# HKU-BAL/MegaPath

Hardware: NVIDIA B200
Metric: read pairs aligned/sec (higher is better)
Workload: dtype int16/u8 (integer DP, 2-bit FM-index)

## Files before the change

megapath_b200/csrc/mp_align.cu:

```cuda
#include "mp_context.h"
#include "mp_cigar.h"
#include <cub/device/device_scan.cuh>
#include <algorithm>
#include <tuple>
#include <string.h>
#include <stdlib.h>

int mps_upload(mp_context *ctx, const uint32_t *queries, const uint32_t *readLengths, uint32_t nReads, uint32_t wpq);
int mps_download_seedpos(mp_context *ctx, mp_seed_pos **readPos, uint64_t *nReadPos, mp_seed_pos **matePos, uint64_t *nMatePos);


__device__ __forceinline__ void account_work(unsigned long long cells, unsigned long long tasks, unsigned long long *__restrict__ counters)
{
#pragma unroll
    for (int d = 16; d; d >>= 1) { cells += __shfl_xor_sync(0xffffffffu, cells, d); tasks += __shfl_xor_sync(0xffffffffu, tasks, d); }
    if ((threadIdx.x & 31) == 0 && tasks) { atomicAdd(&counters[11], cells); atomicAdd(&counters[12], tasks); }
}

__global__ void k_left_tasks(const mp_candidate *__restrict__ cands, uint32_t n, const uint32_t *__restrict__ lens,
                             uint64_t fullLen, int strandLeft, MpDpTask *__restrict__ tasks, unsigned long long *__restrict__ counters)
{
    uint32_t c = blockIdx.x * blockDim.x + threadIdx.x;
    if (c >= n) { account_work(0, 0, counters); return; }
    mp_candidate ci = cands[c];
// ... 494 lines not shown

extern "C" int mp_align_pairs(mp_context *ctx, const mp_align_params *params, mp_results *out)
{
    if (!ctx || !params || !out) { mp_set_error("mp_align_pairs: null argument"); return MP_ERR_ARG; }
    if (!ctx->hasIndex || !ctx->hasBatch) { mp_set_error("mp_align_pairs: index and batch must be loaded first"); return MP_ERR_STATE; }
    if (params->matchScore != 1 || params->extendGapScore != -1 || params->mismatchScore > -2 || params->mismatchScore <= params->openGapScore * 2 ||
        params->mismatchScore < -4 || params->openGapScore < -6 || params->openGapScore >= -1) {
        mp_set_error("mp_align_pairs: score parameters outside the supported range (CPU_DP.cpp:199-208; mismatch = -1 divides by zero at CPU_DP.cpp:310, and for mismatch == 2 * open the reference traceback prefers I over D where the plain recurrence ties: unpinned, refused)"); return MP_ERR_ARG;
    }
    if ((int64_t)ctx->maxLenBatch >= (int64_t)params->maxReadLength) {
        mp_set_error("the batch holds a read of %u bases but maxReadLength is %d (reads must be shorter)", ctx->maxLenBatch, params->maxReadLength);
        return MP_ERR_ARG;
    }
    MP_CUDA(cudaSetDevice(ctx->device));
    const double wall0 = mp_now_ms();
    MpTrace tr;
    memset(out, 0, sizeof *out);
    ctx->resValid = false; ctx->fmtReady = false;
    ctx->hPairs.clear(); ctx->hRescued.clear(); ctx->hSingles.clear(); ctx->hCigars.clear();
    ctx->evUsed = 0;
    MP_CUDA(cudaEventRecord(ctx->ev[4], ctx->stream));
    if (!ctx->seeded) { if (int rc = mp_seed_pairs(ctx, params)) return rc; }
    MP_CUDA(cudaEventRecord(ctx->ev[5], ctx->stream));
    tr.mark("seed_pairs");
    uint64_t cells = 0, tasksRun = 0;
    if (int rc = deep_dp(ctx, params, out, cells, tasksRun)) return rc;
    tr.mark("deep_dp");
    if (int rc = mps_single_and_rescue(ctx, params, out, cells, tasksRun)) return rc;
    MP_CUDA(cudaEventRecord(ctx->ev[6], ctx->stream));
    unsigned long long hc[16];
    MP_CUDA(cudaMemcpyAsync(hc, ctx->dCounters.p, sizeof hc, cudaMemcpyDeviceToHost, ctx->stream));
    MP_CUDA(cudaStreamSynchronize(ctx->stream));
    tr.mark("single+default dp");
    mp_stats &S = ctx->stats;
    memset(&S, 0, sizeof S);
    S.n_occ = hc[2]; S.n_lf = hc[5] + hc[8]; S.n_sa = hc[3]; S.n_lkt = hc[4]; S.n_probe = hc[9]; S.n_text = hc[10];
    ctx->ev_collect(S.ms_fill, S.ms_tb, S.ms_exact);
    S.dp_cells = cells; S.dp_tasks = tasksRun; S.dp_tasks_exact = hc[14]; S.dp_cells_filled = hc[15];
    cudaEventElapsedTime(&S.ms_seed, ctx->ev[0], ctx->ev[1]);
    cudaEventElapsedTime(&S.ms_sa, ctx->ev[1], ctx->ev[2]);
    cudaEventElapsedTime(&S.ms_pair, ctx->ev[2], ctx->ev[3]);
    cudaEventElapsedTime(&S.ms_dp, ctx->ev[5], ctx->ev[6]);
    cudaEventElapsedTime(&S.ms_total, ctx->ev[4], ctx->ev[6]);
    out->pairs = ctx->hPairs.data(); out->n_pairs = ctx->hPairs.size();
    out->rescued = ctx->hRescued.data(); out->n_rescued = ctx->hRescued.size();
    out->singles = ctx->hSingles.data(); out->n_singles = ctx->hSingles.size();
    out->cigars = ctx->hCigars.data(); out->cigar_bytes = ctx->hCigars.size();
    ctx->seeded = false;
    ctx->resCount[0] = out->n_pairs; ctx->resCount[1] = out->n_rescued; ctx->resCount[2] = out->n_singles; ctx->resValid = true;
    if (ctx->resultsOnDevice) {
        out->pairs = nullptr; out->rescued = nullptr; out->singles = nullptr; out->cigars = nullptr;
        out->n_pairs = out->n_rescued = out->n_singles = out->cigar_bytes = 0;
    }
    S.ms_wall = (float)(mp_now_ms() - wall0);
    tr.mark("finish");
    return 0;
}
extern "C" int mp_results_on_device(mp_context *ctx, int on)
{
    if (!ctx) { mp_set_error("mp_results_on_device: null argument"); return MP_ERR_ARG; }
    ctx->resultsOnDevice = on != 0;
    return 0;
}
extern "C" int mp_last_stats(mp_context *ctx, mp_stats *stats)
{
    if (!ctx || !stats) { mp_set_error("mp_last_stats: null argument"); return MP_ERR_ARG; }
// ... 11 lines not shown
```

megapath_b200/csrc/mp_dp.cu:

```cuda
#include "mp_context.h"
#include "mp_cigar.h"
#include <cub/device/device_scan.cuh>
#include <algorithm>
#include <type_traits>

#ifndef MP_FILL_MINBLOCKS
#define MP_FILL_MINBLOCKS 6
#endif
#define DP_BIAS   0x4000
#define DP_BIAS2  0x40004000u
#define DP_NEG2   0x20C020C0u
#define DP_C      0x5000
#define DP_C2     0x50005000u
#define DP_CM1_2  0x4FFF4FFFu

__device__ __forceinline__ int h0_value(int j, int clipLt, int open)
{
    return j <= clipLt ? 0 : open - (j - clipLt - 1);
}
__device__ __forceinline__ uint32_t pack2(int v) { return ((uint32_t)v & 0xffffu) * 0x00010001u; }
__device__ __forceinline__ uint32_t prmt(uint32_t a, uint32_t b, uint32_t sel)
{
    uint32_t d; asm("prmt.b32 %0, %1, %2, %3;" : "=r"(d) : "r"(a), "r"(b), "r"(sel)); return d;
}
// ... 303 lines not shown
#pragma unroll 1
        for (int t = 1; t <= stepsR; ) {
            if (t > rampEnd && t <= steadyEnd) {
#pragma unroll 1
                for (; t <= steadyEnd; t += 4) group(t, std::false_type());
            } else { group(t, std::true_type()); t += 4; }
        }
    }
    __syncwarp();
#pragma unroll
    for (int half = 0; half < 2; ++half) {
        const int lb = tr.lb[half], thr = tr.thr[half];
        int gbest = lb;
#pragma unroll
        for (int dlt = 16; dlt; dlt >>= 1) gbest = max(gbest, __shfl_xor_sync(0xffffffffu, gbest, dlt));
        uint32_t key = 0xffffffffu, c2 = 0u;
        if (lb == gbest && gbest >= thr && tr.elig[half])
            dp_resolve_lane<K>(tables + (size_t)(blockIdx.x * 8 + (threadIdx.x >> 5) * 2) * tableStride + half * 128, S, (int)(threadIdx.x & 31) * K + 1, tr.elig[half], tr.rfirst[half], tr.rlast[half], (gbest - DP_BIAS) >> 2, key, c2);
#ifdef MP_DEBUG_TRACK
        if (pairId == 0 && half == 0) printf("dbg lane %d lb %d gbest %d thr %d thrT %d elig %x r0 %d r1 %d T2 %x N %d L %d partial %d key %x\n", lane, lb, gbest, thr, tr.thrT[0], tr.elig[0], tr.rfirst[0], tr.rlast[0], T2, NA, LA, (int)partial, key);
        if (lb == gbest && gbest >= thr && tr.elig[half] && (key == 0xffffffffu || tr.rfirst[half] < 1 || tr.rlast[half] > (half ? NB : NA)))
            printf("track: pair %u half %d lane %d gbest %d thr %d lb %d r0 %d r1 %d N %d L %d elig %x key %x cnt %u partial %d\n", pairId, half, lane, gbest, thr, lb,
                   tr.rfirst[half], tr.rlast[half], half ? NB : NA, half ? LB : LA, tr.elig[half], key, c2, (int)partial);
#endif
#pragma unroll
        for (int dlt = 16; dlt; dlt >>= 1) { key = min(key, __shfl_xor_sync(0xffffffffu, key, dlt)); c2 += __shfl_xor_sync(0xffffffffu, c2, dlt); }
        if (lane == 0 && (half == 0 || hasB)) {
            FillOut f; f.score = (gbest - DP_BIAS) >> 2; f.row = key >> 12; f.col = key & 0xfffu; f.cnt = c2;
            if (gbest < thr || !(half ? okB : okA) || key == 0xffffffffu) { f.score = 0; f.row = 0; f.col = 0; f.cnt = 0; }
            fill[half == 0 ? tA : tB] = f;
        }
    }
}

template <int K, bool WORDPAT>
__global__ void __launch_bounds__(128)
k_dp_tb(const uint8_t *__restrict__ refSeq, const uint32_t *__restrict__ refLens, uint32_t refStride,
        const uint8_t *__restrict__ readSeq, const uint32_t *__restrict__ readLens, uint32_t readStride,
        const int32_t *__restrict__ cutoffs, uint32_t taskBase, uint32_t nTasks, MpDpParams P,
        const uint8_t *__restrict__ tables, size_t tableStride, int S, const FillOut *__restrict__ fill,
        MpDpOut *__restrict__ outs, uint8_t *__restrict__ patterns, uint32_t patStride,
        const uint32_t *__restrict__ active, const uint32_t *__restrict__ nActive)
{
    const uint32_t lt = blockIdx.x * blockDim.x + threadIdx.x;
    if (active) nTasks = *nActive;
    if (lt >= nTasks) return;
    const uint32_t task = taskBase + (active ? active[lt] : lt);
    const int L = (int)readLens[task], cutoff = cutoffs[task];
    const int mm = P.mismatch, open = P.open, ext = -1, clipLt = P.clipLt;
    MpDpOut o; memset(&o, 0, sizeof o);
    const FillOut f = fill[task];
    if (cutoff > L || cutoff <= 0 || L >= 255 + open - 1 + cutoff || L > 32 * K || f.score < cutoff) { outs[task] = o; return; }
    const uint8_t *tab = tables + (size_t)(lt & ~1u) * tableStride + (lt & 1u) * 128;
    uint8_t *pat = patterns + (size_t)task * patStride;
    uint32_t tabW = 0; size_t tabIdx = ~(size_t)0;
    auto cellAt = [&](int r, int c) -> uint32_t {
        const size_t off = cell_offset<K>(r, c, S);
        if ((off >> 2) != tabIdx) { tabIdx = off >> 2; tabW = __ldcs((const uint32_t *)tab + tabIdx); }
        return (tabW >> ((off & 3) * 8)) & 0xffu;
    };
    auto flagAt = [&](int r, int c) -> int {
        if (c == 0) return 0;
        if (r == 0) return c <= clipLt ? 0 : 1;
        return trace_flag(cellAt(r, c));
    };
    auto hmodAt = [&](int r, int c) -> int {
        if (r == 0) return h0_value(c, clipLt, open) & 63;
        if (c == 0) return 0;
        return trace_h(cellAt(r, c));
    };
    const size_t rsOff = (size_t)task * readStride, fsOff = (size_t)task * refStride;
    uint32_t rsW = 0, fsW = 0; size_t rsIdx = ~(size_t)0, fsIdx = ~(size_t)0;
    auto readBase = [&](int x) -> uint32_t {
        const size_t a = rsOff + x;
        if ((a >> 2) != rsIdx) { rsIdx = a >> 2; rsW = __ldg((const uint32_t *)readSeq + rsIdx); }
        return (rsW >> ((a & 3) * 8)) & 0xffu;
    };
    auto refBase = [&](int x) -> uint32_t {
        const size_t a = fsOff + x;
        if ((a >> 2) != fsIdx) { fsIdx = a >> 2; fsW = __ldg((const uint32_t *)refSeq + fsIdx); }
        return (fsW >> ((a & 3) * 8)) & 0xffu;
    };
    uint32_t p = 0, pacc = 0;
    auto emit = [&](uint32_t byte) {
        if (WORDPAT) {
            pacc |= byte << ((p & 3) * 8);
            if ((p & 3) == 3) { ((uint32_t *)pat)[p >> 2] = pacc; pacc = 0; }
        } else pat[p] = (uint8_t)byte;
        ++p;
    };
    int cgType = 'N', cgCnt = 0, cgLast = 'N', cgLen = 0, cgI = 0, cgD = 0, cgS = 0, cgGap = 0;
    bool cgStored = P.cigText != 0;
    uint8_t *cw = pat + patStride;
    auto cgFlush = [&]() {
        if (cgCnt > 0 && cgType != 'N') {
            const int nd = ndigits(cgCnt);
            cgLen += nd + 1;
            if (cgType == 'I') cgI += cgCnt; else if (cgType == 'D') cgD += cgCnt; else if (cgType == 'S') cgS += cgCnt;
            if (cgType == 'I' || cgType == 'D') cgGap += open + (cgCnt - 1) * ext;
            if (cgStored) {
                if (cw - (nd + 1) < pat + p + 8) cgStored = false;
                else { *--cw = (uint8_t)cgType; int v = cgCnt; for (int d = 0; d < nd; ++d) { *--cw = (uint8_t)('0' + v % 10); v /= 10; } }
            }
        }
    };
    auto cgEvent = [&](int type, int cnt) { if (type == cgType) cgCnt += cnt; else { cgFlush(); cgType = type; cgCnt = cnt; } };
    auto sym = [&](uint32_t ch) { emit(ch); cgEvent((int)ch, 1); cgLast = (int)ch; };
    auto rep = [&](uint32_t c) { emit('V'); emit(c & 0xffu); cgEvent(cgLast, (int)(c & 0xffu) - 1); };
    const int hitRow = (int)f.row, hitCol = (int)f.col;
    o.score = f.score; o.count = min(f.cnt, 255u);
    int clipR = L - hitCol;
    if (clipR > 0) { sym('S'); rep((uint32_t)clipR); }
    int i = L - clipR, j = hitRow;
    enum { NORMAL, I_EXT, D_EXT, SM_EXIT, SI_EXIT, SD_EXIT };
    int state = NORMAL;
    int accum = 0;
    uint32_t cell = cellAt(j, i);
    while (i > 0 && j > 0) {
        const int flag = trace_flag(cell), hcur = trace_h(cell);
        if (state == NORMAL) {
            uint32_t diagCell = 0; int dflag, hdiag;
            if (i - 1 == 0) { dflag = 0; hdiag = 0; }
            else if (j - 1 == 0) { dflag = (i - 1) <= clipLt ? 0 : 1; hdiag = h0_value(i - 1, clipLt, open) & 63; }
            else { diagCell = cellAt(j - 1, i - 1); dflag = trace_flag(diagCell); hdiag = trace_h(diagCell); }
            const int dd = trace_diff(hcur, hdiag);
            bool eq = refBase(j - 1) == readBase(i - 1);
            int ms = eq ? 1 : mm;
            if (dd == ms) {
                if (i != 1 && dflag == 0) { state = SM_EXIT; break; }
                sym(eq ? 'M' : 'm'); --j; --i;
                cell = diagCell;
                continue;
            } else if (flag == 1) {
                int vd = trace_diff(hcur, hmodAt(j - 1, i));
                sym('D'); --j;
                if (vd != open) { accum = (int8_t)(vd - ext); state = D_EXT; }
            } else {
                int hd = trace_diff(hcur, hmodAt(j, i - 1));
                sym('I'); --i;
                if (hd != open) { accum = (int8_t)(hd - ext); state = I_EXT; }
            }
        } else if (state == D_EXT) {
            int vd = trace_diff(hcur, hmodAt(j - 1, i));
            if (vd + accum == open && flagAt(j - 1, i) == 0) { state = SD_EXIT; break; }
            sym('D'); --j;
            if (vd + accum == open) state = NORMAL; else accum = (int8_t)(accum + vd - ext);
        } else {
            int hd = trace_diff(hcur, hmodAt(j, i - 1));
            if (hd + accum == open && flagAt(j, i - 1) == 0) { state = SI_EXIT; break; }
            sym('I'); --i;
            if (hd + accum == open) state = NORMAL; else accum = (int8_t)(accum + hd - ext);
        }
        if (i > 0 && j > 0) cell = cellAt(j, i);
    }
    bool discard = false;
    if (j == 0) {
        int sc = min(clipLt & 0xff, i);
        if (sc < i) { sym('I'); rep((uint32_t)(i - sc)); }
        sym('S'); rep((uint32_t)sc);
    } else if (state == SI_EXIT) {
        sym('I'); sym('S'); rep((uint32_t)(i - 1));
    } else if (state == SD_EXIT) {
        sym('D'); sym('S'); rep((uint32_t)(i - 1));
        discard = true;
    } else if (state == SM_EXIT) {
        sym((refBase(j - 1) == readBase(i - 1)) ? 'M' : 'm');
        sym('S'); rep((uint32_t)(i - 1));
        j -= 1;
    }
    o.patLen = p;
    emit(0);
    if (WORDPAT && (p & 3)) ((uint32_t *)pat)[p >> 2] = pacc;
    cgFlush();
    if (cw < pat + p + 8) cgStored = false;
    o.cigLen = (uint16_t)cgLen; o.nI = (uint16_t)cgI; o.nD = (uint16_t)cgD; o.nS = (uint16_t)cgS; o.gapPenalty = (int16_t)cgGap; o.cigStored = cgStored ? 1 : 0;
    if (discard) { o.score = 0; o.hitLoc = 0; } else o.hitLoc = (uint32_t)j;
    outs[task] = o;
}

template <int K>
__global__ void __launch_bounds__(128)
k_dp_exact(const uint8_t *__restrict__ refSeq, const uint32_t *__restrict__ refLens, uint32_t refStride,
           const uint8_t *__restrict__ readSeq, const uint32_t *__restrict__ readLens, uint32_t readStride,
           const int32_t *__restrict__ cutoffs, uint32_t taskBase, uint32_t nTasks, MpDpParams P,
           MpDpOut *__restrict__ outs, uint8_t *__restrict__ patterns, uint32_t patStride, uint32_t *__restrict__ needDp)
{
    const int lane = threadIdx.x & 31;
    const uint32_t lt = blockIdx.x * 4 + (threadIdx.x >> 5);
    if (lt >= nTasks) return;
    const uint32_t task = taskBase + lt;
    const int N = (int)refLens[task], L = (int)readLens[task], cutoff = cutoffs[task];
    const bool ok = !(cutoff > L || cutoff <= 0 || L >= 255 + P.open - 1 + cutoff || L > 32 * K) && L > 0 && N >= L &&
                    P.mismatch <= 0 && P.open <= 0;
    uint32_t occ = 0; int first = -1;
    if (ok) {
        const uint8_t *fs = refSeq + (size_t)task * refStride, *rs = readSeq + (size_t)task * readStride;
        const int shifts = N - L + 1;
        const int PRE = L < 8 ? L : 8;
        for (int base = 0; base < shifts; base += 32) {
            const int o = base + lane;
            bool alive = o < shifts;
#pragma unroll
            for (int k = 0; k < 8; ++k)
                if (alive && k < PRE) alive = fs[o + k] == rs[k];
            uint32_t cand = __ballot_sync(0xffffffffu, alive);
            while (cand) {
                const int oc = base + __ffs(cand) - 1;
                cand &= cand - 1;
                bool same = true;
                for (int k = PRE + lane; k < L; k += 32) same = same && fs[oc + k] == rs[k];
                if (__all_sync(0xffffffffu, same)) { if (first < 0) first = oc; ++occ; }
            }
        }
    }
    if (occ == 0) { if (lane == 0) needDp[lt] = 1; return; }
    uint8_t *pat = patterns + (size_t)task * patStride;
    for (int k = lane; k < L; k += 32) pat[k] = 'M';
    if (lane == 0) {
        uint32_t p = (uint32_t)L;
        if (first == 0) { pat[p++] = 'S'; pat[p++] = 'V'; pat[p++] = 0; }
        pat[p] = 0;
        MpDpOut o; memset(&o, 0, sizeof o);
        o.score = L; o.hitLoc = (uint32_t)first; o.count = min(occ, 255u); o.patLen = p;
        const int nd = ndigits(L);
        if (P.cigText && p + 8 + nd + 1 <= patStride) {
            uint8_t *cw = pat + patStride; *--cw = 'M';
            int v = L; for (int d = 0; d < nd; ++d) { *--cw = (uint8_t)('0' + v % 10); v /= 10; }
            o.cigStored = 1;
        }
        o.cigLen = (uint16_t)(nd + 1);
        outs[task] = o;
        needDp[lt] = 0;
    }
}
__global__ void k_dp_compact(const uint32_t *__restrict__ needDp, const uint32_t *__restrict__ pos, uint32_t nTasks, uint32_t taskBase,
                             const uint32_t *__restrict__ refLens, const uint32_t *__restrict__ readLens,
                             uint32_t *__restrict__ active, unsigned long long *__restrict__ counters)
{
    const uint32_t t = blockIdx.x * blockDim.x + threadIdx.x;
    unsigned long long cells = 0; uint32_t exact = 0;
    if (t < nTasks) {
        if (needDp[t]) { active[pos[t]] = t; cells = (unsigned long long)refLens[taskBase + t] * readLens[taskBase + t]; }
        else exact = 1;
    }
    cells = __reduce_add_sync(0xffffffffu, (uint32_t)cells);
    exact = __reduce_add_sync(0xffffffffu, exact);
    if ((threadIdx.x & 31) == 0 && counters) { if (cells) atomicAdd(&counters[15], cells); if (exact) atomicAdd(&counters[14], (unsigned long long)exact); }
}

__global__ void k_extract(MpIndexView ix, const uint32_t *__restrict__ reads, uint32_t wpq, const MpDpTask *__restrict__ tasks,
                          uint32_t nTasks, uint8_t *__restrict__ refSeq, uint32_t refStride, uint8_t *__restrict__ readSeq,
                          uint32_t readStride, uint32_t *__restrict__ refLens, uint32_t *__restrict__ readLens, int32_t *__restrict__ cutoffs,
                          int16_t *__restrict__ hints)
{
    const uint32_t task = blockIdx.x;
    if (task >= nTasks) return;
    MpDpTask tk = tasks[task];
    if (!tk.valid || tk.refLen > refStride || tk.readLen > readStride) { tk.refLen = 0; tk.valid = 0; }
    const uint32_t *rd = reads + (size_t)tk.readID * wpq;
    if (((refStride | readStride) & 3u) == 0) {
        uint32_t *fo = (uint32_t *)(refSeq + (size_t)task * refStride), *ro = (uint32_t *)(readSeq + (size_t)task * readStride);
        for (uint32_t a = threadIdx.x * 4; a < tk.refLen; a += blockDim.x * 4) {
            const uint64_t p = tk.refStart + a;
            const uint32_t x = ((uint32_t)__ldg(ix.pac + (p >> 2)) << 8) | __ldg(ix.pac + (p >> 2) + 1);
            const uint32_t v = (x >> (8 - 2 * (uint32_t)(p & 3))) & 0xFFu;
            fo[a >> 2] = (v >> 6) | (((v >> 4) & 3u) << 8) | (((v >> 2) & 3u) << 16) | ((v & 3u) << 24);
// ... 26 lines not shown
    }
    if (threadIdx.x == 0) { refLens[task] = tk.refLen; readLens[task] = tk.valid ? tk.readLen : 0; cutoffs[task] = tk.cutoff; hints[task] = tk.valid ? tk.diag : (int16_t)-1; }
}

static int launch_dp(mp_context *ctx, const uint8_t *dRef, const uint32_t *dRefLens, uint32_t refStride,
                     const uint8_t *dRead, const uint32_t *dReadLens, uint32_t readStride, const int32_t *dCutoffs,
                     uint32_t nTasks, uint32_t maxRefLen, uint32_t maxReadLen, const MpDpParams &Pin,
                     MpDpOut *dOuts, uint8_t *dPatterns, uint32_t patStride, const int16_t *dHints)
{
    if (nTasks == 0) return 0;
    MpDpParams P = Pin;
    if (const char *e = getenv("MP_CIG_TEXT")) if (e[0] == '0') P.cigText = 0;
    const int K = maxReadLen <= 160 ? 5 : maxReadLen <= 256 ? 8 : 10;
    if (maxReadLen > 320) { mp_set_error("read length %u exceeds the DP kernel bound 320", maxReadLen); return MP_ERR_ARG; }
    if ((size_t)4 * (((size_t)maxRefLen + 44) & ~(size_t)3) * sizeof(uint2) > 200 * 1024) {
        mp_set_error("DP window of %u reference bases exceeds the shared-memory staging of the fill kernel (max ~6300)", maxRefLen); return MP_ERR_CAPACITY;
    }
    const int S = ((int)maxRefLen + 44) & ~3;
    const size_t tableStride = (size_t)S * 32 * K;
    if (ctx->dFill.reserve((size_t)nTasks * sizeof(FillOut))) return MP_ERR_CUDA;
    const size_t typical = nTasks >= (1u << 15) ? (size_t)(1u << 18) * tableStride : (size_t)(nTasks + 1) * tableStride;
    const size_t ideal = std::max<size_t>((size_t)(nTasks + 1) * tableStride, typical);
    if (ctx->dTable.cap < ideal) {
        size_t freeB = 0, totalB = 0; cudaMemGetInfo(&freeB, &totalB);
        const size_t maxBytes = std::min<size_t>((size_t)24 << 30, (freeB + ctx->dTable.cap) / 2);
        const size_t want = std::min<size_t>(ideal, maxBytes);
        if (ctx->dTable.cap < want && ctx->dTable.reserve(want)) return MP_ERR_CUDA;
    }
    const uint32_t per = (uint32_t)std::min<size_t>(nTasks, (ctx->dTable.cap / tableStride) & ~(size_t)1);
    if (per == 0) { mp_set_error("not enough device memory for the DP traceback tables"); return MP_ERR_CUDA; }
    uint8_t *tab = ctx->dTable.as<uint8_t>();
    FillOut *fill = ctx->dFill.as<FillOut>();
    const size_t smem = (size_t)4 * S * sizeof(uint2);
    static const bool useExact = !(getenv("MP_DP_EXACT") && getenv("MP_DP_EXACT")[0] == '0');
    const bool rowMaxOk = (int)maxReadLen - P.clipRt - 1 < 30;
    const uint32_t perMax = std::min<uint32_t>(per, nTasks);
    if (useExact && (ctx->dExFlag.reserve(((size_t)perMax + 1) * 4) || ctx->dExPos.reserve(((size_t)perMax + 1) * 4) ||
                     ctx->dExIdx.reserve(((size_t)perMax + 1) * 4) || ctx->dCounters.reserve(16 * 8))) return MP_ERR_CUDA;
    for (uint32_t base = 0; base < nTasks; base += per) {
        const uint32_t n = std::min<uint32_t>(per, nTasks - base);
        dim3 gridF((n + 7) / 8), gridT((n + 127) / 128), block(128);
        const uint32_t *active = nullptr, *nActive = nullptr;
#define LAUNCH_EXACT(KK) do { \
        cudaEvent_t stop_ = ctx->ev_begin(2); \
        MP_CUDA(cudaMemsetAsync(ctx->dExFlag.p, 0, ((size_t)n + 1) * 4, ctx->stream)); \
        (++g_mp_launches), k_dp_exact<KK><<<(n + 3) / 4, block, 0, ctx->stream>>>(dRef, dRefLens, refStride, dRead, dReadLens, readStride, dCutoffs, \
            base, n, P, dOuts, dPatterns, patStride, ctx->dExFlag.as<uint32_t>()); \
        { size_t tb_ = 0; cub::DeviceScan::ExclusiveSum(nullptr, tb_, ctx->dExFlag.as<uint32_t>(), ctx->dExPos.as<uint32_t>(), (int64_t)n + 1, ctx->stream); \
          if (ctx->dScanTmp.reserve(tb_)) return MP_ERR_CUDA; \
          cub::DeviceScan::ExclusiveSum(ctx->dScanTmp.p, tb_, ctx->dExFlag.as<uint32_t>(), ctx->dExPos.as<uint32_t>(), (int64_t)n + 1, ctx->stream); } \
        (++g_mp_launches), k_dp_compact<<<(n + 255) / 256, 256, 0, ctx->stream>>>(ctx->dExFlag.as<uint32_t>(), ctx->dExPos.as<uint32_t>(), n, base, \
            dRefLens, dReadLens, ctx->dExIdx.as<uint32_t>(), ctx->dCounters.as<unsigned long long>()); \
        active = ctx->dExIdx.as<uint32_t>(); nActive = ctx->dExPos.as<uint32_t>() + n; \
        ctx->ev_end(stop_); } while (0)
#define LAUNCH(KK) do { \
        if (useExact) LAUNCH_EXACT(KK); \
        cudaEvent_t stop_ = ctx->ev_begin(0); \
        if (P.mismatch == -2 && P.open == -3 && rowMaxOk) { \
            if (smem > 48 * 1024) MP_CUDA(cudaFuncSetAttribute(k_dp_fill<KK, -2, -3, false>, cudaFuncAttributeMaxDynamicSharedMemorySize, (int)smem)); \
            (++g_mp_launches), k_dp_fill<KK, -2, -3, false><<<gridF, block, smem, ctx->stream>>>(dRef, dRefLens, refStride, dRead, dReadLens, readStride, dCutoffs, dHints, \
                base, n, P, tab, tableStride, S, fill, active, nActive, 1u); \
        } else if (P.mismatch == -2 && P.open == -3) { \
            if (smem > 48 * 1024) MP_CUDA(cudaFuncSetAttribute(k_dp_fill<KK, -2, -3, true>, cudaFuncAttributeMaxDynamicSharedMemorySize, (int)smem)); \
            (++g_mp_launches), k_dp_fill<KK, -2, -3, true><<<gridF, block, smem, ctx->stream>>>(dRef, dRefLens, refStride, dRead, dReadLens, readStride, dCutoffs, dHints, \
                base, n, P, tab, tableStride, S, fill, active, nActive, 1u); \
        } else { \
            if (smem > 48 * 1024) MP_CUDA(cudaFuncSetAttribute(k_dp_fill<KK, 0, 0, true>, cudaFuncAttributeMaxDynamicSharedMemorySize, (int)smem)); \
            (++g_mp_launches), k_dp_fill<KK, 0, 0, true><<<gridF, block, smem, ctx->stream>>>(dRef, dRefLens, refStride, dRead, dReadLens, readStride, dCutoffs, dHints, \
                base, n, P, tab, tableStride, S, fill, active, nActive, 1u); \
        } \
        ctx->ev_end(stop_); stop_ = ctx->ev_begin(1); \
        if ((patStride & 3) == 0 && ((uintptr_t)dPatterns & 3) == 0) \
            (++g_mp_launches), k_dp_tb<KK, true><<<gridT, block, 0, ctx->stream>>>(dRef, dRefLens, refStride, dRead, dReadLens, readStride, dCutoffs, \
                base, n, P, tab, tableStride, S, fill, dOuts, dPatterns, patStride, active, nActive); \
        else \
            (++g_mp_launches), k_dp_tb<KK, false><<<gridT, block, 0, ctx->stream>>>(dRef, dRefLens, refStride, dRead, dReadLens, readStride, dCutoffs, \
                base, n, P, tab, tableStride, S, fill, dOuts, dPatterns, patStride, active, nActive); \
        ctx->ev_end(stop_); } while (0)
        if (K == 5) LAUNCH(5); else if (K == 8) LAUNCH(8); else LAUNCH(10);
#undef LAUNCH
#undef LAUNCH_EXACT
        MP_CUDA(cudaGetLastError());
    }
    return 0;
}

int mpd_run_explicit(mp_context *ctx, const uint8_t *dRef, const uint32_t *dRefLens, uint32_t maxRefLen,
                     const uint8_t *dRead, const uint32_t *dReadLens, uint32_t maxReadLen, const int32_t *dCutoffs,
                     uint32_t nTasks, const MpDpParams &P, MpDpOut *dOuts, uint8_t *dPatterns, uint32_t patStride)
{
    const int16_t *dHints = nullptr;
    if (const char *e = getenv("MP_DP_TEST_HINT")) {
        std::vector<int16_t> h(nTasks, (int16_t)atoi(e));
        if (ctx->dHintTest.reserve((size_t)nTasks * 2)) return MP_ERR_CUDA;
        MP_CUDA(cudaMemcpyAsync(ctx->dHintTest.p, h.data(), (size_t)nTasks * 2, cudaMemcpyHostToDevice, ctx->stream));
        MP_CUDA(cudaStreamSynchronize(ctx->stream));
        dHints = ctx->dHintTest.as<int16_t>();
    }
    return launch_dp(ctx, dRef, dRefLens, maxRefLen, dRead, dReadLens, maxReadLen, dCutoffs, nTasks, maxRefLen, maxReadLen, P,
                     dOuts, dPatterns, patStride, dHints);
}

int mpd_run_tasks(mp_context *ctx, const MpDpTask *dTasks, uint32_t nTasks, uint32_t maxRefLen, uint32_t maxReadLen,
                  const MpDpParams &P, MpDpOut *dOuts, uint8_t *dPatterns, uint32_t patStride)
{
// ... 15 lines not shown
```

Baseline: 38.24 million.

## Resolve near-ungapped DP tasks with bit-parallel diagonal scan before full fill

Replaces the exact-occurrence prefilter kernel with a warp-level ungapped aligner. It builds bit-planes of the reference in shared memory, scores every diagonal via popcount/ffs over mismatch masks, and certifies that no short gapped alignment within a small loss budget could beat the best diagonal. Tasks it certifies get their pattern and CIGAR written directly and skip the banded DP fill and traceback. The cost is extra per-task scanning and shared memory, plus correctness risk in the certification logic; a test env var to skip DP and a Python oracle are also added.

Measured after the change: 39.48 million (median of 6 runs). 1.03x the previous value.

```diff
diff --git a/megapath_b200/csrc/mp_align.cu b/megapath_b200/csrc/mp_align.cu
--- a/megapath_b200/csrc/mp_align.cu
+++ b/megapath_b200/csrc/mp_align.cu
@@ -550,6 +550,8 @@
     MP_CUDA(cudaMemcpyAsync(hc, ctx->dCounters.p, sizeof hc, cudaMemcpyDeviceToHost, ctx->stream));
     MP_CUDA(cudaStreamSynchronize(ctx->stream));
     tr.mark("single+default dp");
+    if (tr.on) fprintf(stderr, "[mp_trace] dp tasks without the table: %llu exact occurrences, %llu ungapped with differences\n",
+                       hc[14] - hc[13], hc[13]);
     mp_stats &S = ctx->stats;
     memset(&S, 0, sizeof S);
     S.n_occ = hc[2]; S.n_lf = hc[5] + hc[8]; S.n_sa = hc[3]; S.n_lkt = hc[4]; S.n_probe = hc[9]; S.n_text = hc[10];
diff --git a/megapath_b200/csrc/mp_dp.cu b/megapath_b200/csrc/mp_dp.cu
--- a/megapath_b200/csrc/mp_dp.cu
+++ b/megapath_b200/csrc/mp_dp.cu
@@ -359,6 +359,57 @@
         }
     }
 }
+
+template <bool WORDPAT>
+struct PatWriter {
+    uint8_t *pat, *cw;
+    int open;
+    static constexpr int ext = -1;
+    uint32_t p = 0, pacc = 0;
+    int cgType = 'N', cgCnt = 0, cgLast = 'N', cgLen = 0, cgI = 0, cgD = 0, cgS = 0, cgGap = 0;
+    bool cgStored;
+    __device__ PatWriter(uint8_t *pat_, uint32_t patStride, int open_, bool cigText) : pat(pat_), cw(pat_ + patStride), open(open_), cgStored(cigText) {}
+    __device__ void emit(uint32_t byte)
+    {
+        if (WORDPAT) {
+            pacc |= byte << ((p & 3) * 8);
+            if ((p & 3) == 3) { ((uint32_t *)pat)[p >> 2] = pacc; pacc = 0; }
+        } else pat[p] = (uint8_t)byte;
+        ++p;
+    }
+    __device__ void cgFlush()
+    {
+        if (cgCnt > 0 && cgType != 'N') {
+            const int nd = ndigits(cgCnt);
+            cgLen += nd + 1;
+            if (cgType == 'I') cgI += cgCnt; else if (cgType == 'D') cgD += cgCnt; else if (cgType == 'S') cgS += cgCnt;
+            if (cgType == 'I' || cgType == 'D') cgGap += open + (cgCnt - 1) * ext;
+            if (cgStored) {
+                if (cw - (nd + 1) < pat + p + 8) cgStored = false;
+                else { *--cw = (uint8_t)cgType; int v = cgCnt; for (int d = 0; d < nd; ++d) { *--cw = (uint8_t)('0' + v % 10); v /= 10; } }
+            }
+        }
+    }
+    __device__ void cgEvent(int type, int cnt) { if (type == cgType) cgCnt += cnt; else { cgFlush(); cgType = type; cgCnt = cnt; } }
+    __device__ void sym(uint32_t ch) { emit(ch); cgEvent((int)ch, 1); cgLast = (int)ch; }
+    __device__ void rep(uint32_t c) { emit('V'); emit(c & 0xffu); cgEvent(cgLast, (int)(c & 0xffu) - 1); }
+    __device__ void run(uint32_t ch, int n)
+    {
+        emit(ch); cgEvent((int)ch, n); cgLast = (int)ch;
+        for (--n; WORDPAT && n > 0 && (p & 3); --n) emit(ch);
+        if (WORDPAT) for (; n >= 4; n -= 4, p += 4) ((uint32_t *)pat)[p >> 2] = ch * 0x01010101u;
+        for (; n > 0; --n) emit(ch);
+    }
+    __device__ void finish(MpDpOut &o)
+    {
+        o.patLen = p;
+        emit(0);
+        if (WORDPAT && (p & 3)) ((uint32_t *)pat)[p >> 2] = pacc;
+        cgFlush();
+        if (cw < pat + p + 8) cgStored = false;
+        o.cigLen = (uint16_t)cgLen; o.nI = (uint16_t)cgI; o.nD = (uint16_t)cgD; o.nS = (uint16_t)cgS; o.gapPenalty = (int16_t)cgGap; o.cigStored = cgStored ? 1 : 0;
+    }
+};
 
 template <int K, bool WORDPAT>
 __global__ void __launch_bounds__(128)
@@ -408,32 +459,9 @@
         if ((a >> 2) != fsIdx) { fsIdx = a >> 2; fsW = __ldg((const uint32_t *)refSeq + fsIdx); }
         return (fsW >> ((a & 3) * 8)) & 0xffu;
     };
-    uint32_t p = 0, pacc = 0;
-    auto emit = [&](uint32_t byte) {
-        if (WORDPAT) {
-            pacc |= byte << ((p & 3) * 8);
-            if ((p & 3) == 3) { ((uint32_t *)pat)[p >> 2] = pacc; pacc = 0; }
-        } else pat[p] = (uint8_t)byte;
-        ++p;
-    };
-    int cgType = 'N', cgCnt = 0, cgLast = 'N', cgLen = 0, cgI = 0, cgD = 0, cgS = 0, cgGap = 0;
-    bool cgStored = P.cigText != 0;
-    uint8_t *cw = pat + patStride;
-    auto cgFlush = [&]() {
-        if (cgCnt > 0 && cgType != 'N') {
-            const int nd = ndigits(cgCnt);
-            cgLen += nd + 1;
-            if (cgType == 'I') cgI += cgCnt; else if (cgType == 'D') cgD += cgCnt; else if (cgType == 'S') cgS += cgCnt;
-            if (cgType == 'I' || cgType == 'D') cgGap += open + (cgCnt - 1) * ext;
-            if (cgStored) {
-                if (cw - (nd + 1) < pat + p + 8) cgStored = false;
-                else { *--cw = (uint8_t)cgType; int v = cgCnt; for (int d = 0; d < nd; ++d) { *--cw = (uint8_t)('0' + v % 10); v /= 10; } }
-            }
-        }
-    };
-    auto cgEvent = [&](int type, int cnt) { if (type == cgType) cgCnt += cnt; else { cgFlush(); cgType = type; cgCnt = cnt; } };
-    auto sym = [&](uint32_t ch) { emit(ch); cgEvent((int)ch, 1); cgLast = (int)ch; };
-    auto rep = [&](uint32_t c) { emit('V'); emit(c & 0xffu); cgEvent(cgLast, (int)(c & 0xffu) - 1); };
+    PatWriter<WORDPAT> pw(pat, patStride, open, P.cigText != 0);
+    auto sym = [&](uint32_t ch) { pw.sym(ch); };
+    auto rep = [&](uint32_t c) { pw.rep(c); };
     const int hitRow = (int)f.row, hitCol = (int)f.col;
     o.score = f.score; o.count = min(f.cnt, 255u);
     int clipR = L - hitCol;
@@ -495,70 +523,252 @@
         sym('S'); rep((uint32_t)(i - 1));
         j -= 1;
     }
-    o.patLen = p;
-    emit(0);
-    if (WORDPAT && (p & 3)) ((uint32_t *)pat)[p >> 2] = pacc;
-    cgFlush();
-    if (cw < pat + p + 8) cgStored = false;
-    o.cigLen = (uint16_t)cgLen; o.nI = (uint16_t)cgI; o.nD = (uint16_t)cgD; o.nS = (uint16_t)cgS; o.gapPenalty = (int16_t)cgGap; o.cigStored = cgStored ? 1 : 0;
+    pw.finish(o);
     if (discard) { o.score = 0; o.hitLoc = 0; } else o.hitLoc = (uint32_t)j;
     outs[task] = o;
 }
 
-template <int K>
+#define UG_MAX_LOSS 5
+__device__ __forceinline__ uint32_t ug_bits(int lo, int hi)
+{
+    lo = max(lo, 0); hi = min(hi, 32);
+    if (hi <= lo) return 0u;
+    return (hi == 32 ? 0xffffffffu : (1u << hi) - 1u) & ~((1u << lo) - 1u);
+}
+template <int W>
+__device__ __forceinline__ void ug_mask(const uint32_t *pl, int SW, const uint32_t (&rlo)[W], const uint32_t (&rhi)[W], int o, int L, uint32_t (&X)[W])
+{
+#pragma unroll
+    for (int w = 0; w < W; ++w) {
+        const int q = 32 * w + o + 32, i = q >> 5, sh = q & 31;
+        const uint32_t flo = __funnelshift_r(pl[i], pl[i + 1], sh), fhi = __funnelshift_r(pl[SW + i], pl[SW + i + 1], sh);
+        const uint32_t fno = __funnelshift_r(pl[2 * SW + i], pl[2 * SW + i + 1], sh);
+        X[w] = ((rlo[w] ^ flo) | (rhi[w] ^ fhi) | fno) & ug_bits(0, L - 32 * w);
+    }
+}
+__device__ __forceinline__ uint32_t ug_word(const uint32_t *pl, int SW, uint32_t rlo, uint32_t rhi, int o, int w, int L)
+{
+    const int q = 32 * w + o + 32, i = q >> 5, sh = q & 31;
+    const uint32_t flo = __funnelshift_r(pl[i], pl[i + 1], sh), fhi = __funnelshift_r(pl[SW + i], pl[SW + i + 1], sh);
+    const uint32_t fno = __funnelshift_r(pl[2 * SW + i], pl[2 * SW + i + 1], sh);
+    return ((rlo ^ flo) | (rhi ^ fhi) | fno) & ug_bits(0, L - 32 * w);
+}
+template <int W>
+__device__ __forceinline__ int ug_first_from(const uint32_t (&X)[W], int a, int L)
+{
+    int r = L;
+#pragma unroll
+    for (int w = W - 1; w >= 0; --w) { const uint32_t x = X[w] & ug_bits(a - 32 * w, 32); if (x) r = 32 * w + __ffs(x) - 1; }
+    return r;
+}
+template <int W>
+__device__ __forceinline__ int ug_last_upto(const uint32_t (&X)[W], int b)
+{
+    int r = -1;
+#pragma unroll
+    for (int w = 0; w < W; ++w) { const uint32_t x = X[w] & ug_bits(0, b + 1 - 32 * w); if (x) r = 32 * w + 31 - __clz(x); }
+    return r;
+}
+
+template <int K, bool WORDPAT>
+__device__ __forceinline__ bool ug_task(const uint8_t *__restrict__ refSeq, const uint32_t *__restrict__ refLens, uint32_t refStride,
+                                        const uint8_t *__restrict__ readSeq, const uint32_t *__restrict__ readLens, uint32_t readStride,
+                                        const int32_t *__restrict__ cutoffs, uint32_t task, const MpDpParams &P, int maxLoss,
+                                        MpDpOut *__restrict__ outs, uint8_t *__restrict__ patterns, uint32_t patStride, uint32_t *pl, int SW,
+                                        uint32_t &need)
+{
+    constexpr int W = K;
+    const int lane = threadIdx.x & 31;
+    const int N = (int)refLens[task], L = (int)readLens[task], cutoff = cutoffs[task];
+    const int mm = P.mismatch, open = P.open, clipLt = P.clipLt, clipRt = P.clipRt;
+    need = 1;
+    if (cutoff > L || cutoff <= 0 || L >= 255 + open - 1 + cutoff || L > 32 * K || L <= 0 || N <= 0 || mm > 0 || open > 0) return false;
+    const uint8_t *fs = refSeq + (size_t)task * refStride, *rs = readSeq + (size_t)task * readStride;
+    for (int s0 = 0; s0 < SW; s0 += 4) {
+        uint32_t b[4];
+#pragma unroll
+        for (int u = 0; u < 4; ++u) { const int p = 32 * (s0 + u - 1) + lane; b[u] = p >= 0 && p < N ? fs[p] : 4u; }
+#pragma unroll
+        for (int u = 0; u < 4; ++u) {
+            const uint32_t lo = __ballot_sync(0xffffffffu, b[u] & 1u), hi = __ballot_sync(0xffffffffu, b[u] & 2u), no = __ballot_sync(0xffffffffu, b[u] > 3u);
+            if (lane == 0 && s0 + u < SW) { pl[s0 + u] = lo; pl[SW + s0 + u] = hi; pl[2 * SW + s0 + u] = no; }
+        }
+    }
+    uint32_t rlo[W], rhi[W], bad = 0;
+#pragma unroll
+    for (int w = 0; w < W; ++w) {
+        const int p = 32 * w + lane;
+        const uint32_t b = p < L ? rs[p] : 0u;
+        rlo[w] = __ballot_sync(0xffffffffu, b & 1u); rhi[w] = __ballot_sync(0xffffffffu, b & 2u); bad |= __ballot_sync(0xffffffffu, b > 3u);
+    }
+    __syncwarp();
+    if (bad) return false;
+    const int minCol = max(L - clipRt, 1), oMin = -UG_MAX_LOSS, oMax = N - L + UG_MAX_LOSS;
+    const int h = L / 2;
+    int wA = (h / 2) >> 5, wB = ((h + L - 2) / 2) >> 5;
+    uint32_t sAlo = 0, sAhi = 0, sBlo = 0, sBhi = 0;
+#pragma unroll
+    for (int w = 0; w < W; ++w) { if (w == wA) { sAlo = rlo[w]; sAhi = rhi[w]; } if (w == wB) { sBlo = rlo[w]; sBhi = rhi[w]; } }
+    int fmin = 1 << 20, fmax = -(1 << 20);
+    int bv = -(1 << 20), bn = 0; uint32_t bkey = 0xffffffffu; int bo = 0, bc = 0, bR = 0;
+    for (int ob = oMin; ob <= oMax; ob += 32) {
+        const int o = ob + lane;
+        if (o > oMax) continue;
+        {
+            const uint32_t xa = ug_word(pl, SW, sAlo, sAhi, o, wA, L), xb = ug_word(pl, SW, sBlo, sBhi, o, wB, L);
+            const bool firstHalf = (xa & ug_bits(2 - 32 * wA, h - 32 * wA)) | (xb & ug_bits(2 - 32 * wB, h - 32 * wB));
+            const bool secondHalf = (xa & ug_bits(h - 32 * wA, L - 2 - 32 * wA)) | (xb & ug_bits(h - 32 * wB, L - 2 - 32 * wB));
+            const int core = __popc(xa & ug_bits(5 - 32 * wA, L - 5 - 32 * wA)) + (wB != wA ? __popc(xb & ug_bits(5 - 32 * wB, L - 5 - 32 * wB)) : 0);
+            if (firstHalf && secondHalf && core > 1) continue;
+        }
+        uint32_t X[W];
+        ug_mask<W>(pl, SW, rlo, rhi, o, L, X);
+        int tot = 0; uint32_t firstHalf = 0, secondHalf = 0;
+#pragma unroll
+        for (int w = 0; w < W; ++w) {
+            tot += __popc(X[w]);
+            firstHalf |= X[w] & ug_bits(2 - 32 * w, h - 32 * w);
+            secondHalf |= X[w] & ug_bits(h - 32 * w, L - 2 - 32 * w);
+        }
+        if (!firstHalf || !secondHalf) { fmin = min(fmin, o); fmax = max(fmax, o); }
+        const int lo = max(0, -o), hi = min(L, N - o);
+        if (tot > 2 * UG_MAX_LOSS + 1 || hi < lo + 1) continue;
+        int U = o >= 0 ? 0 : h0_value(lo, clipLt, open), R = (o < 0 && lo <= clipLt) ? lo : 0, c = lo;
+        auto consider = [&](int v, int col) {
+            const uint32_t key = ((uint32_t)(col + o) << 12) | (uint32_t)col;
+            if (v > bv) { bv = v; bn = 1; bkey = key; bo = o; bc = col; bR = R; }
+            else if (v == bv) { ++bn; if (key < bkey) { bkey = key; bo = o; bc = col; bR = R; } }
+        };
+        auto runTo = [&](int e) {
+            if (e > c) { if (e >= max(c + 1, minCol)) consider(U + e - c, e); U += e - c; c = e; }
+        };
+#pragma unroll
+        for (int w = 0; w < W; ++w) {
+            uint32_t x = X[w] & ug_bits(lo - 32 * w, hi - 32 * w);
+            while (x) {
+                const int m = 32 * w + __ffs(x);
+                x &= x - 1;
+                runTo(m - 1);
+                const int raw = U + mm;
+                if (m <= clipLt && raw < 0) { U = 0; R = m; } else U = raw;
+                if (m >= minCol) consider(U, m);
+                c = m;
+            }
+        }
+        runTo(hi);
+    }
+    int gv = bv;
+#pragma unroll
+    for (int d = 16; d; d >>= 1) gv = max(gv, __shfl_xor_sync(0xffffffffu, gv, d));
+    uint32_t gkey = bv == gv ? bkey : 0xffffffffu; int gn = bv == gv ? bn : 0;
+#pragma unroll
+    for (int d = 16; d; d >>= 1) { gkey = min(gkey, __shfl_xor_sync(0xffffffffu, gkey, d)); gn += __shfl_xor_sync(0xffffffffu, gn, d); }
+    const int D1 = L - gv;
+    if (gv < cutoff || D1 > maxLoss) return false;
+#pragma unroll
+    for (int d = 16; d; d >>= 1) { fmin = min(fmin, __shfl_xor_sync(0xffffffffu, fmin, d)); fmax = max(fmax, __shfl_xor_sync(0xffffffffu, fmax, d)); }
+    if (D1 >= 3 && fmin <= fmax) {
+        bool hit = false;
+        const int cMin = max(oMin, fmin - 3), cMax = min(oMax, fmax + 3);
+        for (int ob = cMin; ob <= cMax; ob += 28) {
+            const int o = ob + lane - 1;
+            const bool valid = o >= cMin && o <= cMax;
+            uint32_t X[W];
+            ug_mask<W>(pl, SW, rlo, rhi, o, L, X);
+            int Pa[3]; uint32_t Qp = 0x3fffffffu;
+#pragma unroll
+            for (int a = 0; a < 3; ++a) Pa[a] = ug_first_from<W>(X, a, L);
+            if (valid) {
+                Qp = 0;
+#pragma unroll
+                for (int k = 0; k < 3; ++k) Qp |= (uint32_t)(ug_last_upto<W>(X, L - 1 - k) + 2) << (10 * k);
+            }
+            const bool own = valid && lane >= 1 && lane <= 28;
+#pragma unroll
+            for (int g = 1; g <= UG_MAX_LOSS - 2; ++g) {
+                const uint32_t qd = __shfl_down_sync(0xffffffffu, Qp, g);
+                const uint32_t qi = __shfl_up_sync(0xffffffffu, Qp, g);
+                if (!own) continue;
+#pragma unroll
+                for (int ins = 0; ins < 2; ++ins) {
+                    const int cost = ins ? 2 * g + 2 : g + 2, o2 = ins ? o - g : o + g;
+                    if (cost > D1) continue;
+                    const uint32_t q = ins ? qi : qd;
+#pragma unroll
+                    for (int a = 0; a < 3; ++a) {
+                        if (a > clipLt || a + o < 0) continue;
+#pragma unroll
+                        for (int k = 0; k < 3; ++k) {
+                            const int b = L - k, Q = (int)((q >> (10 * k)) & 1023u);
+                            if (a + k + cost > D1 || k > clipRt || b < 1 || b + o2 > N) continue;
+                            if (ins) hit |= max(max(a, 1 - o), Q - 1 - g) <= min(Pa[a], b - g);
+                            else hit |= max(max(a, 1), Q - 1) <= min(Pa[a], b);
+                        }
+                    }
+                }
+            }
+        }
+        if (__any_sync(0xffffffffu, hit)) return false;
+    }
+    const int win = __ffs(__ballot_sync(0xffffffffu, bv == gv && bkey == gkey)) - 1;
+    const int o = __shfl_sync(0xffffffffu, bo, win), j = __shfl_sync(0xffffffffu, bc, win), R = __shfl_sync(0xffffffffu, bR, win);
+    need = 0;
+    if (lane != 0) return D1 > 0;
+    uint32_t X[W];
+    ug_mask<W>(pl, SW, rlo, rhi, o, L, X);
+    PatWriter<WORDPAT> pw(patterns + (size_t)task * patStride, patStride, open, P.cigText != 0);
+    if (L - j > 0) { pw.sym('S'); pw.rep((uint32_t)(L - j)); }
+    const int stop = R >= 1 ? R : max(0, -o);
+    int c = j;
+#pragma unroll
+    for (int w = W - 1; w >= 0; --w) {
+        uint32_t x = X[w] & ug_bits(stop - 32 * w, j - 32 * w);
+        while (x) {
+            const int k = 31 - __clz(x), m = 32 * w + k + 1;
+            x ^= 1u << k;
+            if (c > m) pw.run('M', c - m);
+            pw.sym('m');
+            c = m - 1;
+        }
+    }
+    if (c > stop) pw.run('M', c - stop);
+    int hitRow;
+    if (R >= 1) { pw.sym('S'); pw.rep((uint32_t)R); hitRow = R + o; }
+    else if (o >= 0) { if (o == 0) { pw.sym('S'); pw.rep(0u); } hitRow = o; }
+    else {
+        const int i = -o, sc = min(clipLt & 0xff, i);
+        if (sc < i) { pw.sym('I'); pw.rep((uint32_t)(i - sc)); }
+        pw.sym('S'); pw.rep((uint32_t)sc);
+        hitRow = 0;
+    }
+    MpDpOut out; memset(&out, 0, sizeof out);
+    out.score = gv; out.count = (uint32_t)min(gn, 255);
+    pw.finish(out);
+    out.hitLoc = (uint32_t)hitRow;
+    outs[task] = out;
+    return D1 > 0;
+}
+template <int K, bool WORDPAT>
 __global__ void __launch_bounds__(128)
-k_dp_exact(const uint8_t *__restrict__ refSeq, const uint32_t *__restrict__ refLens, uint32_t refStride,
-           const uint8_t *__restrict__ readSeq, const uint32_t *__restrict__ readLens, uint32_t readStride,
-           const int32_t *__restrict__ cutoffs, uint32_t taskBase, uint32_t nTasks, MpDpParams P,
-           MpDpOut *__restrict__ outs, uint8_t *__restrict__ patterns, uint32_t patStride, uint32_t *__restrict__ needDp)
-{
-    const int lane = threadIdx.x & 31;
+k_dp_ungapped(const uint8_t *__restrict__ refSeq, const uint32_t *__restrict__ refLens, uint32_t refStride,
+              const uint8_t *__restrict__ readSeq, const uint32_t *__restrict__ readLens, uint32_t readStride,
+              const int32_t *__restrict__ cutoffs, uint32_t taskBase, uint32_t nTasks, MpDpParams P, int maxLoss,
+              MpDpOut *__restrict__ outs, uint8_t *__restrict__ patterns, uint32_t patStride, uint32_t *__restrict__ needDp,
+              int SW, unsigned long long *__restrict__ counters)
+{
+    extern __shared__ uint32_t ugPlanes[];
+    __shared__ uint32_t nUngapped;
+    if (threadIdx.x == 0) nUngapped = 0;
+    __syncthreads();
     const uint32_t lt = blockIdx.x * 4 + (threadIdx.x >> 5);
-    if (lt >= nTasks) return;
-    const uint32_t task = taskBase + lt;
-    const int N = (int)refLens[task], L = (int)readLens[task], cutoff = cutoffs[task];
-    const bool ok = !(cutoff > L || cutoff <= 0 || L >= 255 + P.open - 1 + cutoff || L > 32 * K) && L > 0 && N >= L &&
-                    P.mismatch <= 0 && P.open <= 0;
-    uint32_t occ = 0; int first = -1;
-    if (ok) {
-        const uint8_t *fs = refSeq + (size_t)task * refStride, *rs = readSeq + (size_t)task * readStride;
-        const int shifts = N - L + 1;
-        const int PRE = L < 8 ? L : 8;
-        for (int base = 0; base < shifts; base += 32) {
-            const int o = base + lane;
-            bool alive = o < shifts;
-#pragma unroll
-            for (int k = 0; k < 8; ++k)
-                if (alive && k < PRE) alive = fs[o + k] == rs[k];
-            uint32_t cand = __ballot_sync(0xffffffffu, alive);
-            while (cand) {
-                const int oc = base + __ffs(cand) - 1;
-                cand &= cand - 1;
-                bool same = true;
-                for (int k = PRE + lane; k < L; k += 32) same = same && fs[oc + k] == rs[k];
-                if (__all_sync(0xffffffffu, same)) { if (first < 0) first = oc; ++occ; }
-            }
-        }
-    }
-    if (occ == 0) { if (lane == 0) needDp[lt] = 1; return; }
-    uint8_t *pat = patterns + (size_t)task * patStride;
-    for (int k = lane; k < L; k += 32) pat[k] = 'M';
-    if (lane == 0) {
-        uint32_t p = (uint32_t)L;
-        if (first == 0) { pat[p++] = 'S'; pat[p++] = 'V'; pat[p++] = 0; }
-        pat[p] = 0;
-        MpDpOut o; memset(&o, 0, sizeof o);
-        o.score = L; o.hitLoc = (uint32_t)first; o.count = min(occ, 255u); o.patLen = p;
-        const int nd = ndigits(L);
-        if (P.cigText && p + 8 + nd + 1 <= patStride) {
-            uint8_t *cw = pat + patStride; *--cw = 'M';
-            int v = L; for (int d = 0; d < nd; ++d) { *--cw = (uint8_t)('0' + v % 10); v /= 10; }
-            o.cigStored = 1;
-        }
-        o.cigLen = (uint16_t)(nd + 1);
-        outs[task] = o;
-        needDp[lt] = 0;
-    }
+    if (lt < nTasks) {
+        uint32_t need;
+        const bool ung = ug_task<K, WORDPAT>(refSeq, refLens, refStride, readSeq, readLens, readStride, cutoffs, taskBase + lt, P, maxLoss,
+                                             outs, patterns, patStride, ugPlanes + (threadIdx.x >> 5) * 3 * SW, SW, need);
+        if ((threadIdx.x & 31) == 0) { needDp[lt] = need; if (ung) atomicAdd(&nUngapped, 1u); }
+    }
+    __syncthreads();
+    if (threadIdx.x == 0 && nUngapped && counters) atomicAdd(&counters[13], (unsigned long long)nUngapped);
 }
 __global__ void k_dp_compact(const uint32_t *__restrict__ needDp, const uint32_t *__restrict__ pos, uint32_t nTasks, uint32_t taskBase,
                              const uint32_t *__restrict__ refLens, const uint32_t *__restrict__ readLens,
@@ -651,7 +861,14 @@
     uint8_t *tab = ctx->dTable.as<uint8_t>();
     FillOut *fill = ctx->dFill.as<FillOut>();
     const size_t smem = (size_t)4 * S * sizeof(uint2);
-    static const bool useExact = !(getenv("MP_DP_EXACT") && getenv("MP_DP_EXACT")[0] == '0');
+    const char *eEx = getenv("MP_DP_EXACT"), *eUg = getenv("MP_DP_UNGAPPED");
+    const bool useExact = !(eEx && eEx[0] == '0');
+    const int maxLoss = (eUg && eUg[0] == '0') || P.mismatch != -2 || P.open != -3 ? 0 : UG_MAX_LOSS;
+    const int SW = ((int)maxRefLen + 32 * K + 100) / 32 + 1;
+    const bool wordPat = (patStride & 3) == 0 && ((uintptr_t)dPatterns & 3) == 0;
+    const char *eSkip = getenv("MP_DP_TEST_SKIP_DP");
+    const bool testSkipDp = useExact && eSkip && eSkip[0] == '1';
+    if (testSkipDp) MP_CUDA(cudaMemsetAsync(dOuts, 0, (size_t)nTasks * sizeof(MpDpOut), ctx->stream));
     const bool rowMaxOk = (int)maxReadLen - P.clipRt - 1 < 30;
     const uint32_t perMax = std::min<uint32_t>(per, nTasks);
     if (useExact && (ctx->dExFlag.reserve(((size_t)perMax + 1) * 4) || ctx->dExPos.reserve(((size_t)perMax + 1) * 4) ||
@@ -662,9 +879,17 @@
         const uint32_t *active = nullptr, *nActive = nullptr;
 #define LAUNCH_EXACT(KK) do { \
         cudaEvent_t stop_ = ctx->ev_begin(2); \
-        MP_CUDA(cudaMemsetAsync(ctx->dExFlag.p, 0, ((size_t)n + 1) * 4, ctx->stream)); \
-        (++g_mp_launches), k_dp_exact<KK><<<(n + 3) / 4, block, 0, ctx->stream>>>(dRef, dRefLens, refStride, dRead, dReadLens, readStride, dCutoffs, \
-            base, n, P, dOuts, dPatterns, patStride, ctx->dExFlag.as<uint32_t>()); \
+        const size_t ugSmem = (size_t)4 * 3 * SW * sizeof(uint32_t); \
+        if (wordPat) { \
+            if (ugSmem > 48 * 1024) MP_CUDA(cudaFuncSetAttribute(k_dp_ungapped<KK, true>, cudaFuncAttributeMaxDynamicSharedMemorySize, (int)ugSmem)); \
+            (++g_mp_launches), k_dp_ungapped<KK, true><<<(n + 3) / 4, block, ugSmem, ctx->stream>>>(dRef, dRefLens, refStride, dRead, dReadLens, readStride, \
+                dCutoffs, base, n, P, maxLoss, dOuts, dPatterns, patStride, ctx->dExFlag.as<uint32_t>(), SW, ctx->dCounters.as<unsigned long long>()); \
+        } else { \
+            if (ugSmem > 48 * 1024) MP_CUDA(cudaFuncSetAttribute(k_dp_ungapped<KK, false>, cudaFuncAttributeMaxDynamicSharedMemorySize, (int)ugSmem)); \
+            (++g_mp_launches), k_dp_ungapped<KK, false><<<(n + 3) / 4, block, ugSmem, ctx->stream>>>(dRef, dRefLens, refStride, dRead, dReadLens, readStride, \
+                dCutoffs, base, n, P, maxLoss, dOuts, dPatterns, patStride, ctx->dExFlag.as<uint32_t>(), SW, ctx->dCounters.as<unsigned long long>()); \
+        } \
+        MP_CUDA(cudaMemsetAsync(ctx->dExFlag.as<uint32_t>() + n, 0, 4, ctx->stream)); \
         { size_t tb_ = 0; cub::DeviceScan::ExclusiveSum(nullptr, tb_, ctx->dExFlag.as<uint32_t>(), ctx->dExPos.as<uint32_t>(), (int64_t)n + 1, ctx->stream); \
           if (ctx->dScanTmp.reserve(tb_)) return MP_ERR_CUDA; \
           cub::DeviceScan::ExclusiveSum(ctx->dScanTmp.p, tb_, ctx->dExFlag.as<uint32_t>(), ctx->dExPos.as<uint32_t>(), (int64_t)n + 1, ctx->stream); } \
@@ -674,6 +899,7 @@
         ctx->ev_end(stop_); } while (0)
 #define LAUNCH(KK) do { \
         if (useExact) LAUNCH_EXACT(KK); \
+        if (testSkipDp) break; \
         cudaEvent_t stop_ = ctx->ev_begin(0); \
         if (P.mismatch == -2 && P.open == -3 && rowMaxOk) { \
             if (smem > 48 * 1024) MP_CUDA(cudaFuncSetAttribute(k_dp_fill<KK, -2, -3, false>, cudaFuncAttributeMaxDynamicSharedMemorySize, (int)smem)); \
@@ -689,7 +915,7 @@
                 base, n, P, tab, tableStride, S, fill, active, nActive, 1u); \
         } \
         ctx->ev_end(stop_); stop_ = ctx->ev_begin(1); \
-        if ((patStride & 3) == 0 && ((uintptr_t)dPatterns & 3) == 0) \
+        if (wordPat) \
             (++g_mp_launches), k_dp_tb<KK, true><<<gridT, block, 0, ctx->stream>>>(dRef, dRefLens, refStride, dRead, dReadLens, readStride, dCutoffs, \
                 base, n, P, tab, tableStride, S, fill, dOuts, dPatterns, patStride, active, nActive); \
         else \
diff --git a/oracle/pyungapped.py b/oracle/pyungapped.py
--- /dev/null
+++ b/oracle/pyungapped.py
@@ -0,0 +1,133 @@
+import numpy as np
+
+MAX_LOSS = 5
+CLIP_BUDGET = 2
+
+
+def h0_value(j, clip_lt, gap_open):
+    return 0 if j <= clip_lt else gap_open - (j - clip_lt - 1)
+
+
+def admitted(N, L, cutoff, gap_open):
+    return not (cutoff > L or cutoff <= 0 or L >= 255 + gap_open - 1 + cutoff or L > 320) and L > 0 and N > 0
+
+
+def decide(ref, read, clip_lt=130, clip_rt=130, mismatch=-2, gap_open=-3, cutoff=None, max_loss=MAX_LOSS, certify=True):
+    from oracle.pyoracle import dp_cutoff
+    ref = [int(x) for x in ref]
+    read = [int(x) for x in read]
+    N, L = len(ref), len(read)
+    if cutoff is None:
+        cutoff = dp_cutoff(L)
+    out = dict(accept=False, reason="ok", loss=None, score=0, hit=0, count=0, pattern=b"")
+    if not admitted(N, L, cutoff, gap_open) or mismatch > 0 or gap_open > 0:
+        out["reason"] = "admission"
+        return out
+    if max(read) > 3:
+        out["reason"] = "base"
+        return out
+    if (mismatch, gap_open) != (-2, -3):
+        max_loss = 0
+    min_col = max(L - clip_rt, 1)
+    o_lo, o_hi = -MAX_LOSS, N - L + MAX_LOSS
+
+    def match(o, c):
+        r = c + o
+        return 1 <= r <= N and ref[r - 1] == read[c - 1]
+
+    best, key, cnt, win = None, None, 0, None
+    for o in range(o_lo, o_hi + 1):
+        lo, hi = max(0, -o), min(L, N - o)
+        if hi < lo + 1:
+            continue
+        U = 0 if o >= 0 else h0_value(lo, clip_lt, gap_open)
+        R = lo if (o < 0 and lo <= clip_lt) else 0
+        for c in range(lo + 1, hi + 1):
+            raw = U + (1 if match(o, c) else mismatch)
+            if c <= clip_lt and raw < 0:
+                U, R = 0, c
+            else:
+                U = raw
+            if c >= min_col:
+                k = (c + o, c)
+                if best is None or U > best:
+                    best, key, cnt, win = U, k, 1, (o, c, R)
+                elif U == best:
+                    cnt += 1
+                    if k < key:
+                        key, win = k, (o, c, R)
+    if best is None or best < cutoff:
+        out["reason"] = "cutoff"
+        return out
+    loss = L - best
+    out["loss"] = loss
+    if certify and loss > max_loss:
+        out["reason"] = "loss"
+        return out
+    if certify and loss >= 3 and competitor(ref, read, clip_lt, clip_rt, loss):
+        out["reason"] = "gap"
+        return out
+    o, j, R = win
+    pat = bytearray()
+    if L - j > 0:
+        pat += b"SV" + bytes([(L - j) & 0xFF])
+    stop = R if R >= 1 else max(0, -o)
+    for c in range(j, stop, -1):
+        pat.append(ord("M") if match(o, c) else ord("m"))
+    if R >= 1:
+        pat += b"SV" + bytes([R & 0xFF])
+        hit = R + o
+    elif o >= 0:
+        if o == 0:
+            pat += b"SV\x00"
+        hit = o
+    else:
+        i = -o
+        sc = min(clip_lt & 0xFF, i)
+        if sc < i:
+            pat += b"IV" + bytes([i - sc])
+        pat += b"SV" + bytes([sc])
+        hit = 0
+    out.update(accept=True, score=best, hit=hit, count=min(cnt, 255), pattern=bytes(pat))
+    return out
+
+
+def prefix_reach(ref, read, o, a):
+    N, L = len(ref), len(read)
+    c = a
+    while c < L and 1 <= c + 1 + o <= N and ref[c + o] == read[c]:
+        c += 1
+    return c
+
+
+def suffix_start(ref, read, o, b):
+    N = len(ref)
+    s = b + 1
+    while s > 1 and 1 <= s - 1 + o <= N and ref[s - 2 + o] == read[s - 2]:
+        s -= 1
+    return s
+
+
+def competitor(ref, read, clip_lt, clip_rt, budget):
+    N, L = len(ref), len(read)
+    for o1 in range(-MAX_LOSS, N - L + MAX_LOSS + 1):
+        for g in range(1, budget):
+            for kind, o2, cost in (("D", o1 + g, g + 2), ("I", o1 - g, 2 * g + 2)):
+                if cost > budget:
+                    continue
+                for a in range(CLIP_BUDGET + 1):
+                    if a > clip_lt or a + o1 < 0:
+                        continue
+                    for k in range(CLIP_BUDGET + 1):
+                        b = L - k
+                        if a + k + cost > budget or k > clip_rt or b < 1 or b + o2 > N:
+                            continue
+                        P = prefix_reach(ref, read, o1, a)
+                        Q = suffix_start(ref, read, o2, b)
+                        if kind == "D":
+                            ok = max(a, 1, Q - 1) <= min(P, b)
+                        else:
+                            ok = max(a, 1 - o1, Q - 1 - g) <= min(P, b - g)
+                        if ok:
+                            return True
+    return False
```
